# joelle-o-world/dusp

Measured on AMD Instinct MI355X. Metric: rendered Msamples/sec (whole node) + HBM GB/s fraction, 1024-voice 48kHz, higher is better.
Workload: dtype f64; 1 GPU; configs[2] per-voice: 1024 voices/GPU x Multiply(Osc(10k), Ramp(T,1,0) triggered), 60s @48000 Hz, every voice's PCM written; voices_per_gpu=1024, voices_total=1024, n_samples=2880000, engine=fused, parallelism=voices sharded over 1 GPU(s), no collective

## Files before the change

dusp_amd/csrc/abi_internal.hpp:

```cpp
#pragma once
#include <hip/hip_runtime.h>

#include <algorithm>
#include <cstddef>
#include <cstdint>
#include <exception>
#include <map>
#include <mutex>
#include <new>
#include <stdexcept>
#include <string>
#include <utility>
#include <vector>

#include "../../include/dusp_hip.h"
#include "device_types.hpp"
#include "fused_plan.hpp"
#include "jit_codegen.hpp"
#include "program.hpp"
#include "score_plan.hpp"

namespace dusp {
hipError_t launch_chunk_engine(const ChunkArgs &a, hipStream_t stream);
hipError_t launch_state_init(double *state, const double *init, uint32_t n_slots, uint32_t n_pad, hipStream_t stream);
// ... 113 lines not shown
    DevBuf<int64_t> d_jit_regime;

    static constexpr size_t kCount = 28;

    template <class F>
    void for_each_workspace(F &&f) {
        f("chunk buffers", d_scratch);
        f("rings", d_rings);
        f("unit state", d_state);
        f("segment phases", d_seg);
        f("fused end state", d_fused_state);
        f("voice records", d_recs);
        f("sum-chain records", d_sum_voices);
        f("parked chunks", d_saved_bufs);
        f("parked rings", d_rings_wave);
        f("staging PCM", d_host_out);
        f("staging frames", d_host_frames);
        f("staging PCM frames / peaks", d_host_pcm);
        f("staging PCM frames / peaks", d_host_peaks);
        f("mix sums / gains", d_mix);
        f("mix sums / gains", d_mix_gains);
        f("staging parameters", d_host_par);
        f("staging inputs", d_host_in);
        f("hand-off buffers", d_handoff_init);
        f("hand-off buffers", d_handoff_out);
        f("program constants", d_ops);
        f("program constants", d_out_bufs);
        f("program constants", d_init);
        f("compiled kernel's constants", d_jit_fk);
        f("compiled kernel's constants", d_jit_dk);
        f("compiled kernel's constants", d_jit_scan);
        f("warm-up records", d_warm_records);
        f("warm-up start state", d_warm_init);
        f("column verdicts", d_jit_regime);
    }
    const char *first_overwritten() {
        const char *hit = nullptr;
        for_each_workspace([&](const char *name, auto &buf) {
            if (!hit && !buf.intact()) hit = name;
        });
        return hit;
    }
};
static_assert(sizeof(dusp_workspaces) == dusp_workspaces::kCount * sizeof(DevBuf<char>), "dusp_workspaces holds DevBufs only: update kCount and for_each_workspace");

struct dusp_program : dusp_workspaces {
    dusp_ctx *ctx = nullptr;
    dusp::Program P;
    int engine = DUSP_ENGINE_CHUNK;
    dusp::FusedPlan fused;
    dusp::WavePlan wave;
    std::vector<dusp::SumVoice> h_sum_voices;
    std::vector<double> h_sum_end;
    uint32_t last_n_inst = 0, last_n_pad = 0;
    bool rendered = false;
    std::vector<double> h_state;
    bool h_state_valid = false;
    bool mixed = false;
    std::vector<unsigned> mix_range;
    uint32_t mix_n_inst = 0;
    int requested_engine = DUSP_ENGINE_AUTO;
    bool resumable = false;
    bool persistent = false;
    bool keep_memory = false;
    bool delay_changed = false;
    bool migrate_to_chunk = false;
    int64_t next_clock = 0;
    hipEvent_t ev0 = nullptr, ev1 = nullptr;
    hipStream_t last_stream = nullptr;
    bool jit_ok = false;
    std::string jit_why;
    std::map<std::pair<int, int>, dusp::JitSource> jit_src;
    bool jit_consts_uploaded = false;
    int voice_loop = -1;
    uint64_t jit_table_generation = 0;
    int jit_waves = 0, jit_per_wave = 0;
    unsigned jit_segments = 1;
    bool jit_voices = false;
    bool jit_scan = false;
    bool handoff_ok = false;
    std::string handoff_why;
    unsigned warm_redo_from = 0;
    unsigned char *pin[1] = {nullptr};
    size_t pin_bytes = 0;

    dusp_program() = default;
    dusp_program(const dusp_program &) = delete;
    dusp_program &operator=(const dusp_program &) = delete;
    ~dusp_program() {
        if (ctx) (void)hipSetDevice(ctx->device);
        for_each_workspace([](const char *, auto &buf) { buf.release(); });
        if (pin[0]) (void)hipHostFree(pin[0]);
        if (ev0) (void)hipEventDestroy(ev0);
        if (ev1) (void)hipEventDestroy(ev1);
    }
};

#define CTX_FAIL(ctx, code, msg)  \
    do {                          \
        (ctx)->err = (msg);       \
        return (code);            \
    } while (0)

#define HIP_TRY(ctx, expr)                                                                        \
    do {                                                                                          \
        hipError_t e_ = (expr);                                                                   \
        if (e_ != hipSuccess) {                                                                   \
            (ctx)->err = std::string("HIP error: ") + hipGetErrorString(e_) + " in " + #expr;     \
            return DUSP_ERR_HIP;                                                                  \
        }                                                                                         \
    } while (0)

template <class F>
int guarded(std::string &err, const char *who, F &&body) noexcept {
    try {
        return body();
    } catch (const std::bad_alloc &) {
        try { err = std::string(who) + ": out of host memory"; } catch (...) {}
        return DUSP_ERR_NOMEM;
    } catch (const std::length_error &e) {
        try { err = std::string(who) + ": size out of range (" + e.what() + ")"; } catch (...) {}
        return DUSP_ERR_ARG;
    } catch (const std::exception &e) {
        try { err = std::string(who) + ": " + e.what(); } catch (...) {}
        return DUSP_ERR_ARG;
    } catch (...) {
        try { err = std::string(who) + ": unknown internal error"; } catch (...) {}
        return DUSP_ERR_ARG;
    }
}

inline bool instances_in_range(size_t n_instances) { return n_instances >= 1 && n_instances <= (1u << 24); }
inline bool samples_in_range(size_t n_samples) { return n_samples >= 1 && n_samples <= (1ull << 31); }
inline bool batch_in_range(size_t n_instances, size_t n_samples) { return instances_in_range(n_instances) && samples_in_range(n_samples); }
inline bool channels_in_range(size_t n_channels) { return n_channels >= 1 && n_channels <= 64; }

inline int check_batch(dusp_ctx *ctx, const char *who, size_t n_instances, size_t n_samples) {
    if (!batch_in_range(n_instances, n_samples)) CTX_FAIL(ctx, DUSP_ERR_ARG, std::string(who) + ": n_instances must be in [1, 2^24] and n_samples in [1, 2^31]");
    return DUSP_OK;
}
inline int check_channels(dusp_ctx *ctx, const char *who, size_t n_channels) {
    if (!channels_in_range(n_channels)) CTX_FAIL(ctx, DUSP_ERR_UNSUPPORTED, std::string(who) + ": the outlet must have 1..64 channels");
    return DUSP_OK;
}
inline int check_pcm_format(dusp_ctx *ctx, const char *who, int format, bool allow_planar) {
    if ((format != 0 || !allow_planar) && format != DUSP_PCM_S16 && format != DUSP_PCM_S24 && format != DUSP_PCM_F32)
        CTX_FAIL(ctx, DUSP_ERR_ARG, std::string(who) + ": format must be " + (allow_planar ? "0 (planar f32), " : "") + "DUSP_PCM_S16 (1), DUSP_PCM_S24 (2) or DUSP_PCM_F32 (3)");
// ... 26 lines not shown
```

dusp_amd/csrc/abi_program.hip:

```cpp
#include <cmath>
#include <cstdio>
#include <cstdlib>
#include <cstring>
#include <memory>

#include "abi_internal.hpp"
#include "engine_select.hpp"
#include "jit_engine.hpp"

extern "C" {

static int select_engine(dusp_program *prog) {
    dusp_ctx *ctx = prog->ctx;
    dusp::EngineRequest rq;
    rq.requested = prog->requested_engine;
    rq.resumable = prog->resumable;
    rq.rendered = prog->rendered;
    rq.engine_so_far = prog->engine;
    rq.delay_changed = prog->delay_changed;
    rq.wave_jit = ctx->knobs.wave_jit;
    for (int k = 0; k < dusp::kNumTables; k++) rq.table_set[k] = ctx->table_set[k], rq.table_fx32_ok[k] = ctx->table_fx32_ok[k];
    dusp::EngineChoice choice = dusp::engine_select(prog->P, rq, std::move(prog->wave.ramp_checked));
    prog->fused = std::move(choice.fused);
    prog->wave = std::move(choice.wave);
    prog->persistent = choice.persistent;
    if (choice.error) CTX_FAIL(ctx, choice.error, choice.error_text);
    prog->engine = choice.engine;
    prog->jit_src.clear();
    prog->jit_consts_uploaded = false;
    prog->jit_ok = choice.jit_ok;
    prog->jit_why = std::move(choice.jit_why);
    prog->handoff_ok = choice.handoff_ok;
    prog->handoff_why = std::move(choice.handoff_why);
    return DUSP_OK;
}

static int upload_constants(dusp_program *prog) {
    dusp_ctx *ctx = prog->ctx;
    HIP_TRY(ctx, hipSetDevice(ctx->device));
    const dusp::Program &P = prog->P;
    size_t n_all_ops = P.ops.size();
    for (const auto &w : P.warm_ops) n_all_ops += w.size();
    HIP_TRY(ctx, prog->d_ops.ensure(n_all_ops));
    std::vector<int32_t> out_bufs = P.out_bufs;
    if (prog->engine == DUSP_ENGINE_WAVE) {
        std::vector<dusp::DevOp> ops = P.ops;
        const auto &slot = prog->wave.buf_slot;
        for (size_t k = 0; k < ops.size(); k++) {
            if (ops[k].out_buf >= 0) ops[k].out_buf = slot[(size_t)ops[k].out_buf];
            for (auto &in : ops[k].in)
                if (in.kind == dusp::SRC_BUF && in.idx >= 0 && in.idx < P.n_bufs) in.idx = slot[(size_t)in.idx];
            ops[k].lds_slot = prog->wave.op_state[k];
        }
        for (auto &op : ops)
            if (op.op == dusp::OP_RETRIGGER) op.pad = prog->wave.op_state[(size_t)op.pad];
        for (auto &b : out_bufs) b = slot[(size_t)b];
        std::vector<dusp::DevOp> ordered(ops.size());
        for (size_t at = 0; at < ops.size(); at++) ordered[at] = ops[(size_t)prog->wave.order[at]];
        HIP_TRY(ctx, hipMemcpy(prog->d_ops.p, ordered.data(), ordered.size() * sizeof(dusp::DevOp), hipMemcpyHostToDevice));
    } else
    HIP_TRY(ctx, hipMemcpy(prog->d_ops.p, P.ops.data(), P.ops.size() * sizeof(dusp::DevOp), hipMemcpyHostToDevice));
    n_all_ops = P.ops.size();
    for (const auto &w : P.warm_ops) {
        if (!w.empty())
            HIP_TRY(ctx, hipMemcpy(prog->d_ops.p + n_all_ops, w.data(), w.size() * sizeof(dusp::DevOp), hipMemcpyHostToDevice));
        n_all_ops += w.size();
    }
    HIP_TRY(ctx, prog->d_out_bufs.ensure(out_bufs.size()));
    HIP_TRY(ctx, hipMemcpy(prog->d_out_bufs.p, out_bufs.data(), out_bufs.size() * sizeof(int32_t), hipMemcpyHostToDevice));
    if (!P.init_state.empty()) {
        HIP_TRY(ctx, prog->d_init.ensure(P.init_state.size()));
        HIP_TRY(ctx, hipMemcpy(prog->d_init.p, P.init_state.data(), P.init_state.size() * sizeof(double), hipMemcpyHostToDevice));
    }
    return DUSP_OK;
}

// ... 44 lines not shown
    const dusp::Program &P = prog->P;
    bool same = next.g.units.size() == P.g.units.size() && next.ops.size() == P.ops.size() && next.n_bufs == P.n_bufs &&
                next.ring_samples == P.ring_samples && next.out_bufs == P.out_bufs && next.g.n_params == P.g.n_params &&
                next.g.sample_rate == P.g.sample_rate && next.init_state.size() == P.init_state.size() &&
                next.dev_rings.size() == P.dev_rings.size();
    for (size_t k = 0; same && k < P.g.units.size(); k++) same = next.g.units[k].op == P.g.units[k].op && next.g.units[k].n_out == P.g.units[k].n_out;
    for (size_t k = 0; same && k < P.ops.size(); k++) {
        const dusp::DevOp &a = P.ops[k], &b = next.ops[k];
        same = a.op == b.op && a.unit == b.unit && a.out_buf == b.out_buf && a.state_slot == b.state_slot && a.ring_base == b.ring_base &&
               a.ring_len == b.ring_len && a.n_in == b.n_in;
        for (int j = 0; same && j < dusp::kMaxIn; j++)
            same = (a.in[j].kind == dusp::SRC_BUF) == (b.in[j].kind == dusp::SRC_BUF) && (a.in[j].kind != dusp::SRC_BUF || a.in[j].idx == b.in[j].idx);
    }
    if (!same) CTX_FAIL(ctx, DUSP_ERR_ARG, "dusp_program_continue: the descriptor does not describe the circuit this program was built from");
    if (next.g.clock0 != prog->next_clock)
        CTX_FAIL(ctx, DUSP_ERR_STATE, "dusp_program_continue: descriptor clock " + std::to_string(next.g.clock0) + " does not follow the rendered clock " +
                                          std::to_string(prog->next_clock));
    const bool persistent = next.ring_samples != 0 || !next.feed_forward;
    if (persistent && !(prog->resumable && (prog->engine == DUSP_ENGINE_CHUNK || prog->engine == DUSP_ENGINE_WAVE)))
        CTX_FAIL(ctx, DUSP_ERR_STATE, "dusp_program_continue: a circuit with delay lines / feedback has to be built with DUSP_ENGINE_RESUMABLE");
    const int engine_before = prog->engine;
    bool delay_changed = prog->delay_changed;
    for (size_t k = 0; k < P.ops.size(); k++)
        if (P.ops[k].op == dusp::OP_DELAY) {
            const dusp::DevOperand &a = P.ops[k].in[1], &b = next.ops[k].in[1];
            if (a.kind != b.kind || a.idx != b.idx || std::memcmp(&a.cval, &b.cval, sizeof(float)) != 0) delay_changed = true;
        }
    struct Before {
        dusp::Program P; bool delay_changed; int engine;
    } before{std::move(prog->P), prog->delay_changed, prog->engine};
    prog->P = std::move(next);
    prog->delay_changed = delay_changed;
    if (int rc = finish_build(prog)) {
        const std::string why = ctx->err;
        prog->P = std::move(before.P);
        prog->delay_changed = before.delay_changed;
        const int requested = prog->requested_engine;
        prog->requested_engine = before.engine;
        const int back = finish_build(prog);
        prog->requested_engine = requested;
        ctx->err = back == DUSP_OK ? why : why + " (and the previous program could not be restored: " + ctx->err + ")";
        return rc;
    }
    prog->keep_memory = persistent;
    if (persistent && engine_before == DUSP_ENGINE_WAVE && prog->engine == DUSP_ENGINE_CHUNK) prog->migrate_to_chunk = true;
    return DUSP_OK;
    });
}

void dusp_program_destroy(dusp_program *prog) {
    if (!prog) return;
    (void)hipSetDevice(prog->ctx->device);
    if (prog->rendered && prog->ev1) (void)hipEventSynchronize(prog->ev1);
    (void)hipStreamSynchronize(prog->ctx->stream);
    delete prog;
}

int dusp_program_info_get(const dusp_program *prog, dusp_program_info *info) {
    if (!prog || !info) return DUSP_ERR_ARG;
    std::memset(info, 0, sizeof *info);
    const dusp::Graph &g = prog->P.g;
    info->sample_rate = (uint32_t)g.sample_rate;
    info->chunk_size = (uint32_t)g.chunk;
    info->n_units = (uint32_t)g.units.size();
    info->n_out_channels = (uint32_t)prog->P.out_bufs.size();
    info->n_params = (uint32_t)g.n_params;
    info->engine = (uint32_t)prog->engine;
    info->n_device_ops = (uint32_t)prog->P.ops.size();
    info->n_inputs = (uint32_t)g.n_inputs;
    if (prog->engine == DUSP_ENGINE_FUSED) std::snprintf(info->shape, sizeof info->shape, "%s", prog->fused.shape.c_str());
    if (prog->engine == DUSP_ENGINE_WAVE && prog->jit_ok && (prog->jit_waves || !prog->rendered))
    {
        const int at = std::snprintf(info->shape, sizeof info->shape, "%s, compiled kernel: %d units, %dx%d", prog->P.feed_forward ? "feed-forward" : "feedback",
                                     (int)prog->P.ops.size(), prog->jit_waves, prog->jit_per_wave);
        if (at > 0 && (size_t)at < sizeof info->shape && (prog->jit_voices || prog->jit_segments > 1)) {
            if (prog->jit_voices && prog->jit_segments > 1) std::snprintf(info->shape + at, sizeof info->shape - (size_t)at, ", loop, %u seg", prog->jit_segments);
            else if (prog->jit_voices) std::snprintf(info->shape + at, sizeof info->shape - (size_t)at, ", voice loop");
            else if (prog->warm_redo_from) std::snprintf(info->shape + at, sizeof info->shape - (size_t)at, ", %u seg, redo@%u", prog->jit_segments, prog->warm_redo_from);
            else std::snprintf(info->shape + at, sizeof info->shape - (size_t)at, ", %u seg", prog->jit_segments);
        } else if (at > 0 && (size_t)at < sizeof info->shape && prog->jit_scan)
            std::snprintf(info->shape + at, sizeof info->shape - (size_t)at, ", scan");
    }
    else if (prog->engine == DUSP_ENGINE_WAVE && prog->jit_ok)
        std::snprintf(info->shape, sizeof info->shape, "%s, %d chunk buffers in LDS (kernel compiling)", prog->P.feed_forward ? "feed-forward" : "feedback", prog->wave.n_slots);
    else if (prog->engine == DUSP_ENGINE_WAVE)
        std::snprintf(info->shape, sizeof info->shape, "%s, %d chunk buffers in LDS", prog->P.feed_forward ? "feed-forward" : "feedback", prog->wave.n_slots);
    if (prog->engine == DUSP_ENGINE_CHUNK && !prog->P.warm_ops.empty() && !prog->handoff_ok && !prog->handoff_why.empty())
        std::snprintf(info->shape, sizeof info->shape, "warm-up, then not compiled: %.34s", prog->handoff_why.c_str());
    if (prog->engine == DUSP_ENGINE_CHUNK && prog->handoff_ok && prog->jit_waves)
        std::snprintf(info->shape, sizeof info->shape, "%d warm-up chunks here, then compiled kernel: %d units, %dx%d", (int)prog->P.warm_ops.size(), (int)prog->P.ops.size(),
                      prog->jit_waves, prog->jit_per_wave);
    return DUSP_OK;
}

int dusp_state_download(dusp_program *prog, size_t instance, size_t unit, double *out, size_t cap) {
    if (!prog) return DUSP_ERR_ARG;
    dusp_ctx *ctx = prog->ctx;
    return guarded(ctx->err, "dusp_state_download", [&]() -> int {
    if (!prog->rendered) CTX_FAIL(ctx, DUSP_ERR_STATE, "dusp_state_download: nothing has been rendered yet");
    if (prog->mixed) CTX_FAIL(ctx, DUSP_ERR_STATE, "dusp_state_download: the last render was a mix (dusp_render_host_mix, dusp_render_host_score): unit state describes its last tile only");
    const dusp::Graph &g = prog->P.g;
    if (unit >= g.units.size() || instance >= prog->last_n_inst || !out)
        CTX_FAIL(ctx, DUSP_ERR_ARG, "dusp_state_download: unit / instance out of range");
    HIP_TRY(ctx, hipSetDevice(ctx->device));
    HIP_TRY(ctx, hipEventSynchronize(prog->ev1));
    const dusp::UnitDesc &u = g.units[unit];
// ... 117 lines not shown
```

dusp_amd/csrc/abi_render.hip:

```cpp
#include <cstring>

#include "abi_internal.hpp"
#include "jit_plan.hpp"
#include "render_plan.hpp"
#include "ring_windows.hpp"

static int check_tables(dusp_program *prog) {
    dusp_ctx *ctx = prog->ctx;
    for (const auto &u : prog->P.g.units)
        if (u.op == dusp::OP_OSC || u.op == dusp::OP_MULTI_OSC || u.op == dusp::OP_SHAPE) {
            const int w = (int)u.attrs[0];
            if (!ctx->d_tables || !ctx->table_set[w])
                CTX_FAIL(ctx, DUSP_ERR_STATE, "render: wave table " + std::to_string(w) + " has not been uploaded (dusp_table_upload)");
            if (ctx->table_len != (uint32_t)prog->P.g.sample_rate + 1)
                CTX_FAIL(ctx, DUSP_ERR_STATE, "render: wave table length != sample_rate + 1");
        }
    return DUSP_OK;
}


hipError_t zero_rings(dusp_program *prog, uint32_t n_pad, uint32_t n_chunks, bool instance_major, hipStream_t stream) {
    const dusp::Program &P = prog->P;
    float *rings = prog->d_rings.p;
    const size_t total = (size_t)P.ring_samples;
// ... 49 lines not shown
    a.table_stride = prog->ctx->table_stride;
    a.flags = flags;
    a.n_warm = (uint32_t)P.warm_ops.size();
    for (uint32_t k = 0, at = a.n_ops; k < a.n_warm; k++) {
        a.warm_first[k] = at;
        a.warm_n[k] = (uint32_t)P.warm_ops[k].size();
        at += a.warm_n[k];
    }
    return a;
}


int check_guards(dusp_program *prog, hipStream_t stream) {
    dusp_ctx *ctx = prog->ctx;
    if (!g_guard_bytes) return DUSP_OK;
    HIP_TRY(ctx, hipStreamSynchronize(stream));
    const char *hit = prog->first_overwritten();
    if (!hit && ctx->tables_guarded && ctx->d_tables && !guard_intact((const char *)ctx->d_tables + sizeof(float) * dusp::kNumTables * ctx->table_stride)) hit = "lookup tables";
    if (hit) CTX_FAIL(ctx, DUSP_ERR_HIP, std::string("render: a kernel wrote past the end of a device buffer (") + hit + "): guard bytes overwritten");
    return DUSP_OK;
}

struct RenderCall {
    uint32_t n_inst, n_chunks, n_pad;
    size_t n_samples;
    const float *d_params, *d_inputs;
    float *d_out;
    hipStream_t stream;
};

static size_t chunk_workspace_floats(const dusp::Program &P, uint32_t rows) { return (size_t)std::max(1, P.n_bufs) * dusp::kChunk * rows; }
static size_t state_workspace_doubles(const dusp::Program &P, uint32_t n_pad) { return std::max<size_t>(1, P.init_state.size()) * n_pad; }
static size_t ring_workspace_floats(const dusp::Program &P, uint32_t n_pad) { return std::max<size_t>(1, (size_t)P.ring_samples) * n_pad; }

static int clear_chunk_memory(dusp_program *prog, uint32_t n_pad, hipStream_t stream) {
    dusp_ctx *ctx = prog->ctx;
    HIP_TRY(ctx, hipMemsetAsync(prog->d_scratch.p, 0, chunk_workspace_floats(prog->P, n_pad) * sizeof(float), stream));
    if (prog->P.ring_samples) HIP_TRY(ctx, hipMemsetAsync(prog->d_rings.p, 0, (size_t)prog->P.ring_samples * n_pad * sizeof(float), stream));
    return DUSP_OK;
}

static int render_sum_chain(dusp_program *prog, const RenderCall &c, dusp::FusedLaunch &L, const ChainWindow *window) {
    dusp_ctx *ctx = prog->ctx;
    const uint32_t n_inst = c.n_inst;
    hipStream_t stream = c.stream;
    if (!L.table_fx32_ok) CTX_FAIL(ctx, DUSP_ERR_UNSUPPORTED, "render: wave table has entries below 2^-20; build this program with DUSP_ENGINE_CHUNK");
    const int gb = dusp::sumchain_group_blocks(n_inst, c.n_samples, ctx->n_cus);
    if (!gb) CTX_FAIL(ctx, DUSP_ERR_UNSUPPORTED, "render: too many samples for the fused sum chain; use DUSP_ENGINE_CHUNK");
    if (window) {
        L.chain_first = window->first;
        L.chain_init = window->init;
        L.chain_raw = window->raw;
    }
    dusp::build_sum_voices(prog->fused, (uint32_t)prog->P.g.sample_rate, gb, L.chain_first + (uint64_t)c.n_chunks * dusp::kChunk, prog->h_sum_voices, prog->h_sum_end);
    HIP_TRY(ctx, prog->d_sum_voices.ensure(prog->h_sum_voices.size()));
    HIP_TRY(ctx, hipMemcpyAsync(prog->d_sum_voices.p, prog->h_sum_voices.data(), prog->h_sum_voices.size() * sizeof(dusp::SumVoice), hipMemcpyHostToDevice, stream));
    std::vector<double> end((size_t)prog->fused.n_state_words * n_inst);
    for (int w = 0; w < prog->fused.n_state_words; w++)
        for (uint32_t i = 0; i < n_inst; i++) end[(size_t)w * n_inst + i] = prog->h_sum_end[(size_t)w];
    HIP_TRY(ctx, hipMemcpyAsync(prog->d_fused_state.p, end.data(), end.size() * sizeof(double), hipMemcpyHostToDevice, stream));
    HIP_TRY(ctx, hipStreamSynchronize(stream));
    HIP_TRY(ctx, hipEventRecord(prog->ev0, stream));
    HIP_TRY(ctx, dusp::launch_sumchain(prog->fused, L, prog->d_sum_voices.p, gb, stream));
    HIP_TRY(ctx, hipEventRecord(prog->ev1, stream));
    return DUSP_OK;
}

static int render_fused(dusp_program *prog, const RenderCall &c, const ChainWindow *window) {
    dusp_ctx *ctx = prog->ctx;
    dusp::FusedLaunch L{};
    L.params = c.d_params;
    L.tables = ctx->d_tables;
    L.table_stride = ctx->table_stride;
    L.out = c.d_out;
    L.n_inst = c.n_inst;
    L.n_samples = c.n_samples;
    L.n_chunks = c.n_chunks;
    L.sample_rate = (uint32_t)prog->P.g.sample_rate;
    L.n_cus = ctx->n_cus;
    L.table_antisym = ctx->table_antisym[prog->fused.table_id];
    L.table_finite = ctx->table_finite[prog->fused.table_id];
    L.table_fx32_ok = ctx->table_fx32_ok[prog->fused.table_id];
    L.table_delta = ctx->table_delta[prog->fused.table_id];
    L.table_form = ctx->table_form[prog->fused.table_id];
    L.knobs = ctx->knobs;
    HIP_TRY(ctx, prog->d_recs.ensure(c.n_inst));
    L.recs = prog->d_recs.p;
    HIP_TRY(ctx, prog->d_fused_state.ensure((size_t)std::max(1, prog->fused.n_state_words) * c.n_inst));
    L.end_state = prog->d_fused_state.p;
    if (prog->fused.kind == dusp::FUSED_SUMCHAIN) {
        if (int rc = render_sum_chain(prog, c, L, window)) return rc;
    } else {
        HIP_TRY(ctx, hipEventRecord(prog->ev0, c.stream));
        HIP_TRY(ctx, dusp::launch_fused(prog->fused, L, c.stream));
        HIP_TRY(ctx, hipEventRecord(prog->ev1, c.stream));
    }
    finish_render(prog, c.n_inst, c.n_pad, c.n_chunks);
    return DUSP_OK;
}

static int render_wave_interpreter(dusp_program *prog, const RenderCall &c) {
    dusp_ctx *ctx = prog->ctx;
    const dusp::Program &P = prog->P;
    const uint32_t n_inst = c.n_inst, n_pad = c.n_pad, n_chunks = c.n_chunks;
    hipStream_t stream = c.stream;
    HIP_TRY(ctx, prog->d_state.ensure(state_workspace_doubles(P, n_pad)));
    dusp::WaveArgs w{};
    w.ops = prog->d_ops.p;
    w.out_bufs = prog->d_out_bufs.p;
    w.params = c.d_params;
    w.tables = ctx->d_tables;
    w.inputs = c.d_inputs;
    w.out = c.d_out;
    w.state = prog->d_state.p;
    w.init_state = prog->d_init.p;
    w.n_samples = c.n_samples;
    w.n_ops = (uint32_t)P.ops.size();
    w.n_out = (uint32_t)P.out_bufs.size();
    w.n_inst = n_inst;
    w.n_pad = n_pad;
    w.n_bufs = (uint32_t)prog->wave.n_slots;
    w.n_state_ops = (uint32_t)prog->wave.n_state_ops;
    w.n_groups = n_chunks;
    w.sample_rate = (uint32_t)P.g.sample_rate;
    w.table_stride = ctx->table_stride;
    w.vec4_ok = (c.n_samples % 4 == 0) && (((uintptr_t)c.d_out & 15) == 0);
    w.lds_table_id = prog->wave.lds_table_id;
    w.clock0 = (uint64_t)P.g.clock0;
    w.has_filter = prog->wave.has_filter ? 1u : 0u;
    w.scratch_bytes = (uint32_t)prog->wave.scratch_bytes;
    w.ring_events = prog->wave.ring_events ? 1u : 0u;
    w.ext_units = (uint32_t)prog->wave.ext_units;
    w.n_params = (uint32_t)P.g.n_params;
    w.ring_samples = (uint64_t)P.ring_samples;
    const bool resume = prog->keep_memory;
    if (resume && n_inst != prog->last_n_inst) CTX_FAIL(ctx, DUSP_ERR_STATE, "render: the instance count cannot change while a program is being continued");
    if (P.ring_samples && !resume) {
        HIP_TRY(ctx, prog->d_rings.ensure(ring_workspace_floats(P, n_pad)));
        HIP_TRY(ctx, zero_rings(prog, n_pad, n_chunks, true, stream));
    }
    w.rings = prog->d_rings.p;
    w.resume = resume ? 1u : 0u;
    w.save_bufs = (prog->resumable && prog->persistent) ? 1u : 0u;
    if (w.save_bufs) {
        HIP_TRY(ctx, prog->d_saved_bufs.ensure(chunk_workspace_floats(P, n_inst)));
// ... 175 lines not shown
```

dusp_amd/csrc/fused_engine.hip:

```cpp
#include <hip/hip_runtime.h>

#include <type_traits>

#include "device_types.hpp"
#include "fused_device.hpp"
#include "fused_plan.hpp"
#include "repeat_add.hpp"

namespace dusp {

namespace {

template <bool FASTDIV>
__device__ __forceinline__ float ramp_value(const FusedArgs &A, double tn, double dy) {
    const double tt = fmin(tn, A.r_d);
    double q;
    if (FASTDIV) {
        q = tt * A.r_rcp;
        const double rem = fma(-q, A.r_d, tt);
        q = fma(rem, A.r_rcp, q);
    } else
        q = tt / A.r_d;
    return (float)(A.r_y0 + q * dy);
}
// ... 13 lines not shown
    for (int c = 1; c < 4; ++c) P[c] = addmod(P[c - 1], rc.Fm, rc.S);
}

}

__global__ void dusp_fused_prepare(FusedArgs A, OscRec *recs) {
    const uint32_t inst = blockIdx.x * blockDim.x + threadIdx.x;
    if (inst >= A.n_inst) return;
    const uint32_t sr = A.sample_rate;
    const double srd = (double)sr;
    OscRec rc;
    double fd = (double)operand_value(A.f, A.params, A.n_inst, inst);
    rc.bad = !(fabs(fd) <= 3.0e38);
    if (rc.bad) fd = 0.0;
    if (fabs(fd) >= srd) fd = fmod(fd, srd);
    int E = 0;
    if (fd != 0.0) E = min(E, lsb_exponent(fd));
    if (A.phase0 != 0.0) E = min(E, lsb_exponent(A.phase0));
    const int Emin = -(62 - (32 - __builtin_clz(sr)));
    if (E < Emin) E = Emin;
    rc.E = E;
    rc.u = ldexp(1.0, E);
    rc.S = (uint64_t)sr << (-E);
    const long long F = (long long)rint(ldexp(fd, -E));
    rc.Fm = F >= 0 ? (uint64_t)F : rc.S - (uint64_t)(-F);
    if (rc.Fm >= rc.S) rc.Fm -= rc.S;
    rc.P0 = (uint64_t)rint(ldexp(A.phase0, -E));
    if (rc.P0 >= rc.S) rc.P0 %= rc.S;
    rc.step4 = mulmod(rc.Fm, 4, rc.S);
    rc.step256 = mulmod(rc.Fm, kChunk, rc.S);
    rc.segstep = mulmod(rc.Fm, (uint64_t)A.seg_groups * kChunk, rc.S);
    rc.gain = A.gain.kind == SRC_PARAM || A.gain.kind == SRC_CONST ? operand_value(A.gain, A.params, A.n_inst, inst) : 1.f;
    rc.pad = 0;
    recs[inst] = rc;

    const uint64_t T_end = (uint64_t)A.n_chunks * kChunk;
    double phase_end = (double)addmod(rc.P0, mulmod(rc.Fm, T_end, rc.S), rc.S) * rc.u;
    if (rc.bad) phase_end = __builtin_nan("");
    A.end_state[(size_t)A.osc_state_word * A.n_inst + inst] = phase_end;
    if (A.ramp_state_word >= 0) {
        const double t_end = A.r_playing ? fmin(A.r_t0 + (double)T_end, A.r_d) : A.r_t0;
        const bool playing_end = A.r_playing && (A.r_t0 + (double)T_end <= A.r_d);
        A.end_state[(size_t)A.ramp_state_word * A.n_inst + inst] = t_end;
        A.end_state[(size_t)(A.ramp_state_word + 1) * A.n_inst + inst] = playing_end ? 1.0 : 0.0;
    }
    if (A.shape_state_word >= 0) {
        const double t_end = A.s_playing ? repeat_add(A.s_t0, A.s_c, T_end) : A.s_t0;
        A.end_state[(size_t)A.shape_state_word * A.n_inst + inst] = t_end;
        A.end_state[(size_t)(A.shape_state_word + 1) * A.n_inst + inst] = A.s_playing ? 1.0 : 0.0;
        A.end_state[(size_t)(A.shape_state_word + 2) * A.n_inst + inst] = (A.s_finished || (T_end > 0 && t_end > srd)) ? 1.0 : 0.0;
    }
}

template <int KIND, int TBL, int R, bool FASTDIV, bool FINITE, int BLOCK>
__global__ void __launch_bounds__(BLOCK) dusp_fused_kernel(FusedArgs A, const OscRec *__restrict__ recs) {
    extern __shared__ __attribute__((aligned(16))) float lds_table[];
    Table<TBL> table;
    table.g = A.table;
    table.h = lds_table;
    table.N = A.sample_rate + 1;
    table.M = A.sample_rate / 2;
    table.form = make_table_form(A.table_form, A.sample_rate);
    if (TBL == 1) load_half_table<BLOCK>(lds_table, A.table, A.sample_rate);
    const uint32_t lane = threadIdx.x & 63u;
    constexpr uint32_t waves_per_block = BLOCK / 64;
    constexpr int RS = R < 4 ? R : 4;
    const uint32_t n_blk = (A.n_inst + R - 1) / R;
    const uint64_t n_items = (uint64_t)n_blk * A.n_seg;
    const uint64_t total_waves = (uint64_t)gridDim.x * waves_per_block;
    const double srd = (double)A.sample_rate;
    const uint32_t sr = A.sample_rate;
    const double dy = A.r_y1 - A.r_y0;
    const uint32_t n_full = A.vec4_ok ? (uint32_t)(A.n_samples / kChunk) : 0u;

    for (uint64_t item = (uint64_t)blockIdx.x * waves_per_block + (threadIdx.x >> 6); item < n_items; item += total_waves) {
        const uint32_t blk = A.seg_major ? (uint32_t)(item / A.n_seg) : (uint32_t)(item % n_blk);
        const uint32_t seg = A.seg_major ? (uint32_t)(item % A.n_seg) : (uint32_t)(item / n_blk);
        const uint32_t g0 = seg * A.seg_groups;
        const uint32_t g1 = min(g0 + A.seg_groups, A.n_groups);
        const uint32_t gm = max(g0, min(g1, n_full));
        const uint64_t t_start = (uint64_t)g0 * kChunk;

        uint32_t inst[R];
        int e_min = 0;
        bool any_bad = false;
#pragma unroll
        for (int r = 0; r < R; ++r) {
            inst[r] = min(blk * R + r, A.n_inst - 1);
            e_min = min(e_min, recs[inst[r]].E);
            any_bad = any_bad || recs[inst[r]].bad;
        }
        float *const row0 = A.out + t_start + lane * 4;
        const double tn0 = A.r_t0 + (A.r_playing ? (double)(t_start + lane * 4 + 1) : 0.0);
        const double tn_step = A.r_playing ? (double)kChunk : 0.0;
        const double tn_c = A.r_playing ? 1.0 : 0.0;
        double tn;
        const double st0 = (KIND == FUSED_OSC_SHAPE && A.s_playing) ? repeat_add(A.s_t0, A.s_c, t_start) : A.s_t0;
        double st;
        auto ramp4 = [&](float (&rv)[4]) {
            if (KIND == FUSED_OSC_SHAPE) {
                if (!A.s_playing) {
#pragma unroll
                    for (int c = 0; c < 4; ++c) rv[c] = shape_value(A, st, srd);
                } else {
                    long long T, ce;
                    int K;
                    if (linear_run(st, A.s_c, kChunk, T, ce, K)) {
                        T += (long long)(lane * 4) * ce;
#pragma unroll
                        for (int c = 0; c < 4; ++c) {
                            T += ce;
                            rv[c] = shape_value(A, ldexp((double)T, K - 52), srd);
                        }
                        st = ldexp((double)(T + (long long)(kChunk - 4 - lane * 4) * ce), K - 52);
                    } else {
                        double t = repeat_add(st, A.s_c, (uint64_t)lane * 4);
#pragma unroll
                        for (int c = 0; c < 4; ++c) rv[c] = shape_value(A, t = t + A.s_c, srd);
                        st = __shfl(t, 63, 64);
                    }
                }
            }
            if (KIND == FUSED_OSC_RAMP) {
                rv[0] = ramp_value<FASTDIV>(A, tn, dy);
#pragma unroll
                for (int c = 1; c < 4; ++c) rv[c] = ramp_value<FASTDIV>(A, tn + tn_c * c, dy);
                tn += tn_step;
            }
// ... 185 lines not shown
                run(gm, g1, std::false_type{});
            }
        } else {
            for (int sub = 0; sub < R; sub += RS) {
                double ph[RS][4], D[RS];
                size_t roff[RS];
                float gain[RS];
                bool bad[RS];
#pragma unroll
                for (int r = 0; r < RS; ++r) {
                    const OscRec rc = recs[inst[sub + r]];
                    uint64_t P[4];
                    start_phase(rc, seg, lane, P);
                    for (int c = 0; c < 4; ++c) ph[r][c] = (double)P[c] * rc.u;
                    D[r] = (double)rc.step256 * rc.u;
                    roff[r] = (size_t)inst[sub + r] * A.n_samples;
                    gain[r] = rc.gain;
                    bad[r] = rc.bad;
                }
                tn = tn0;
            st = st0;
                float *row = row0;
                auto run = [&](uint32_t ga, uint32_t gb, auto vec) {
                    for (uint32_t g = ga; g < gb; ++g) {
                        float rv[4] = {1.f, 1.f, 1.f, 1.f};
                        ramp4(rv);
#pragma unroll
                        for (int r = 0; r < RS; ++r) {
                            float v[4];
#pragma unroll
                            for (int c = 0; c < 4; ++c) {
                                const uint32_t idx = (uint32_t)(int)ph[r][c];
                                const double fraction = ph[r][c] - (double)(int)idx;
                                float ta, tb;
                                table.pair(idx, ta, tb);
                                float x = (float)((double)ta * (1.0 - fraction) + (double)tb * fraction);
                                if (bad[r]) x = 0.f;
                                v[c] = finish(x, rv[c], gain[r]);
                                ph[r][c] += D[r];
                                if (ph[r][c] >= srd) ph[r][c] -= srd;
                            }
                            store4<decltype(vec)::value>(row + roff[r], v, (uint64_t)g * kChunk + lane * 4, A.n_samples);
                        }
                        row += kChunk;
                    }
                };
                run(g0, gm, std::true_type{});
                run(gm, g1, std::false_type{});
            }
        }
    }
}

template <int KIND, int TBL, int R, bool FASTDIV, bool FINITE, int BLOCK>
static hipError_t launch_one(const FusedArgs &A, const OscRec *recs, int grid, size_t lds_bytes, hipStream_t stream) {
    auto kernel = dusp_fused_kernel<KIND, TBL, R, FASTDIV, FINITE, BLOCK>;
    if (lds_bytes > 65536) {
        hipError_t e = hipFuncSetAttribute((const void *)kernel, hipFuncAttributeMaxDynamicSharedMemorySize, (int)lds_bytes);
        if (e != hipSuccess) return e;
    }
    hipLaunchKernelGGL(kernel, dim3((unsigned)grid), dim3(BLOCK), lds_bytes, stream, A, recs);
    return hipGetLastError();
}

hipError_t launch_fused(const FusedPlan &plan, const FusedLaunch &L, hipStream_t stream) {
    FusedArgs A{};
    A.params = L.params;
    A.table = L.tables + (size_t)plan.table_id * L.table_stride;
    A.out = L.out;
    A.end_state = L.end_state;
    A.n_samples = L.n_samples;
    A.n_inst = L.n_inst;
    A.n_groups = (uint32_t)((L.n_samples + kChunk - 1) / kChunk);
    A.sample_rate = L.sample_rate;
    A.n_chunks = L.n_chunks;
    A.f = plan.f;
    A.gain = plan.gain;
    if (plan.kind != FUSED_OSC_GAIN) A.gain.kind = -1;
    A.phase0 = plan.phase0;
    A.r_d = plan.r_d; A.r_y0 = plan.r_y0; A.r_y1 = plan.r_y1; A.r_t0 = plan.r_t0; A.r_rcp = plan.r_rcp;
    A.r_playing = plan.r_playing;
    A.r_fastdiv = plan.r_fastdiv;
    A.vec4_ok = (L.n_samples % 4 == 0) && (((uintptr_t)L.out & 15) == 0);
    A.osc_state_word = 0;
    A.ramp_state_word = plan.kind == FUSED_OSC_RAMP ? 1 : -1;
    A.shape_state_word = plan.kind == FUSED_OSC_SHAPE ? 1 : -1;
    if (plan.kind == FUSED_OSC_SHAPE) {
        A.s_table = L.tables + (size_t)plan.s_table_id * L.table_stride;
        A.s_t0 = plan.s_t0; A.s_c = plan.s_c; A.s_min = plan.s_min; A.s_max = plan.s_max;
        A.s_left = plan.s_left; A.s_right = plan.s_right;
        A.s_left_is_shape = plan.s_left_is_shape; A.s_right_is_shape = plan.s_right_is_shape;
        A.s_playing = plan.s_playing; A.s_finished = plan.s_finished;
    }
    auto ordinary = [](double y) { return y == 0.0 || (std::fabs(y) >= 9.3e-10 && std::fabs(y) <= 1.1e18); };
    A.r_scale_ok = plan.kind == FUSED_OSC_RAMP && ordinary(plan.r_y0) && ordinary(plan.r_y1) && plan.r_d <= 1.1e12 && (plan.r_t0 == 0.0 || plan.r_t0 >= 1.0) &&
                           L.knobs.fused_fx32 != 2
                       ? 1 : 0;
    A.fx32_ok = L.table_fx32_ok && L.knobs.fused_fx32 ? 1 : 0;
    A.table_delta = L.knobs.fused_fx32 == 1 ? L.table_delta : 0;
    A.seg_major = L.knobs.fused_segmajor;

    int tbl = (L.table_antisym && L.sample_rate % 2 == 0) ? 1 : 0;
    if (L.table_form >= TABLE_FORM_SAW && L.table_form <= TABLE_FORM_TRIANGLE) tbl = 2;
    A.table_form = L.table_form;
    if (L.knobs.fused_table_global) tbl = 0;
    const size_t lds_bytes = tbl == 1 ? half_table_lds_bytes(L.sample_rate) : 0;
    if (lds_bytes > 160 * 1024) tbl = 0;

    int R = L.knobs.fused_R;
    if (R != 1 && R != 4 && R != 8) R = 4;
    const int block = tbl == 1 ? 1024 : 256;
    const int grid = tbl == 1 ? L.n_cus : L.n_cus * 8;
    const uint64_t total_waves = (uint64_t)grid * (block / 64);
    const uint64_t n_blk = (A.n_inst + R - 1) / R;
    auto cut = [&](uint64_t per_wave, uint64_t &n_seg) {
// ... 40 lines not shown
```

dusp_amd/csrc/fused_plan.hpp:

```cpp
#pragma once
#include <cmath>
#include <string>
#include <vector>

#include "device_types.hpp"
#include "program.hpp"

namespace dusp {

enum : int { FUSED_OSC = 0, FUSED_OSC_RAMP = 1, FUSED_OSC_GAIN = 2, FUSED_SUMCHAIN = 3, FUSED_OSC_SHAPE = 4 };

struct FusedPlan {
    std::string shape, why;
    int kind = FUSED_OSC;
    int table_id = 0;
    DevOperand f{}, gain{};
    double phase0 = 0;
    double r_d = 1, r_y0 = 0, r_y1 = 0, r_t0 = 0, r_rcp = 1;
    int r_playing = 0, r_fastdiv = 0;
    int s_table_id = 0, s_playing = 0, s_finished = 0, s_left_is_shape = 0, s_right_is_shape = 0;
    double s_t0 = 0, s_c = 0, s_left = 0, s_right = 0;
    float s_min = 0, s_max = 1;
    std::vector<double> sum_f, sum_phase0;
    std::vector<int> sum_units;
    bool sum_all_int = false;
    int sum_env = 0;
    std::vector<float> sum_gain;
    std::vector<int> sum_ramp_units;
    int n_state_words = 0;
    std::vector<int> unit_state_first, unit_state_count;
};

struct OscRec {
    uint64_t S, Fm, P0;
    uint64_t step4, step256, segstep;
    double u;
    int32_t E, bad;
    float gain, pad;
};

struct SumVoice {
    uint64_t B0, bs, step4, step256, Fm;
    float gain;
    uint32_t pad;
};

struct SumArgs {
    const SumVoice *voices;
    const float *table;
    float *out;
    uint64_t n_samples, S;
    double inv_S, inv_sr;
    uint32_t n_voices, n_inst, n_groups, n_blocks, sample_rate, vec4_ok;
    double r_d, r_y0, r_y1, r_t0;
    int32_t r_playing, r_fastdiv;
    const float *init;
    uint32_t first_block, raw;
};

struct WaveArgs {
    const DevOp *ops;
    const int32_t *out_bufs;
    const float *params;
    const float *tables;
    float *out;
    double *state;
    const double *init_state;
    uint64_t n_samples;
    uint32_t n_ops, n_out, n_inst, n_pad, n_bufs, n_groups, sample_rate, table_stride, vec4_ok;
    int32_t lds_table_id;
    uint32_t table_bytes, wave_bytes;
    float *rings;
    uint64_t ring_samples, clock0;
    uint32_t has_filter, scratch_bytes;
    const float *inputs;
    uint32_t n_state_ops;
    uint32_t ring_events;
    uint32_t ext_units;
    uint32_t n_seg, seg_groups;
    uint32_t pass_mode;
    uint32_t pass_level;
    unsigned long long *seg_sum, *seg_start;
    int32_t max_osc_level, pad4;
    float *saved_bufs;
    uint32_t save_bufs, resume;
    uint32_t n_params, param_bytes;
};

inline size_t wave_param_bytes(size_t n_params) { return n_params && n_params <= 2048 ? (n_params * 4 + 15) & ~(size_t)15 : 0; }
inline size_t wave_lds_bytes(size_t n_bufs, size_t n_state_ops, size_t scratch_bytes) {
    return (n_bufs * 1024 + n_state_ops * 96 + (scratch_bytes ? scratch_bytes + 16 : 0) + 15) & ~(size_t)15;
}

struct WavePlan {
    bool ok = false, has_filter = false;
    int scratch_bytes = 0;
    std::vector<int> order;
    std::vector<int> buf_slot;
    std::vector<int> op_state;
    int n_slots = 0, n_state_ops = 0;
    int ext_units = 0;
    bool ring_events = false;
    bool splittable = false;
    bool splittable_but_for_filters = false;
    int max_osc_level = 0;
    std::vector<int> osc_level;
    std::vector<int> ramp_fastdiv;
    struct RampChecked { double d, t0; bool ok; };
    std::vector<RampChecked> ramp_checked;
    int lds_table_id = -1;
    std::string why;
// ... 561 lines not shown
```

dusp_amd/csrc/sumchain_engine.hip:

```cpp
#include <hip/hip_runtime.h>

#include "device_types.hpp"
#include "fused_device.hpp"
#include "fused_plan.hpp"

namespace dusp {

template <int TBL, bool INT, int GB, bool FINITE, int BLOCK, int ENV>
__global__ void __launch_bounds__(BLOCK) dusp_sumchain_kernel(SumArgs A) {
    extern __shared__ __attribute__((aligned(16))) float lds_table[];
    Table<TBL> table;
    table.g = A.table;
    table.h = lds_table;
    table.N = A.sample_rate + 1;
    table.M = A.sample_rate / 2;
    if (TBL == 1) load_half_table<BLOCK>(lds_table, A.table, A.sample_rate);

    const uint32_t lane = threadIdx.x & 63u;
    constexpr uint32_t waves_per_block = BLOCK / 64;
    const uint64_t n_items = (uint64_t)A.n_inst * A.n_blocks;
    const uint64_t total_waves = (uint64_t)gridDim.x * waves_per_block;
    const uint32_t sr = A.sample_rate;
    const uint32_t n_full = A.first_block * GB + (A.vec4_ok ? (uint32_t)(A.n_samples / kChunk) : 0u);

    for (uint64_t item = (uint64_t)blockIdx.x * waves_per_block + (threadIdx.x >> 6); item < n_items; item += total_waves) {
        const uint32_t blk = (uint32_t)(item % A.n_blocks) + A.first_block;
        const uint32_t inst = (uint32_t)(item / A.n_blocks);
        const uint32_t g0 = blk * GB;
        const size_t row_at = (size_t)inst * A.n_samples + (size_t)(g0 - A.first_block * GB) * kChunk + lane * 4;
        float acc[GB][4];
#pragma unroll
        for (int g = 0; g < GB; ++g)
            for (int c = 0; c < 4; ++c) acc[g][c] = 0.f;
        if (A.init) {
#pragma unroll
            for (int g = 0; g < GB; ++g)
                if (g0 + g < n_full) {
                    const f32x4 v = *(const f32x4 *)(A.init + row_at + (size_t)g * kChunk);
                    acc[g][0] = v[0]; acc[g][1] = v[1]; acc[g][2] = v[2]; acc[g][3] = v[3];
                } else if (g0 + g < A.n_groups) {
                    const uint64_t t = (uint64_t)(g0 + g - A.first_block * GB) * kChunk + lane * 4;
                    for (int c = 0; c < 4; ++c)
                        if (t + c < A.n_samples) acc[g][c] = A.init[row_at + (size_t)g * kChunk + c];
                }
        }
        float env[ENV == 2 ? GB : 1][4];
        if (ENV == 2) {
            const double dy = A.r_y1 - A.r_y0, rcp = 1.0 / A.r_d;
#pragma unroll
            for (int g = 0; g < (ENV == 2 ? GB : 1); ++g)
#pragma unroll
                for (int c = 0; c < 4; ++c) {
                    const uint64_t n = (uint64_t)(g0 + g) * kChunk + lane * 4 + c;
                    const double tt = A.r_playing ? fmin(A.r_t0 + (double)(n + 1), A.r_d) : A.r_t0;
                    double q;
                    if (A.r_fastdiv) {
                        q = tt * rcp;
                        q = fma(fma(-q, A.r_d, tt), rcp, q);
                    } else
                        q = tt / A.r_d;
                    env[g][c] = (float)(A.r_y0 + q * dy);
                }
        }

        for (uint32_t j = 0; j < A.n_voices; ++j) {
            const SumVoice rc = A.voices[j];
            if (INT) {
                const uint32_t f = (uint32_t)(rc.Fm >> 32), s4 = (uint32_t)(rc.step4 >> 32), s256 = (uint32_t)(rc.step256 >> 32);
                const uint32_t base = mod_u32((uint32_t)(rc.B0 >> 32) + blk * (uint32_t)(rc.bs >> 32), sr, A.inv_sr);
                uint32_t idx[4];
                idx[0] = mod_u32(base + lane * s4, sr, A.inv_sr);
#pragma unroll
                for (int c = 1; c < 4; ++c) {
                    idx[c] = idx[c - 1] + f;
                    idx[c] = min(idx[c], idx[c] - sr);
                }
#pragma unroll
                for (int g = 0; g < GB; ++g)
#pragma unroll
                    for (int c = 0; c < 4; ++c) {
                        float v = table.at(idx[c]);
                        if (ENV == 1) v = v * rc.gain;
                        if (ENV == 2) v = v * env[g][c];
                        acc[g][c] = acc[g][c] + v;
                        idx[c] += s256;
                        idx[c] = min(idx[c], idx[c] - sr);
                    }
            } else {
                const uint64_t base = mod_u64(rc.B0 + (uint64_t)blk * rc.bs, A.S, A.inv_S);
                uint64_t P = mod_u64(base + (uint64_t)lane * rc.step4, A.S, A.inv_S);
                uint32_t I[4], F[4];
#pragma unroll
                for (int c = 0; c < 4; ++c) {
                    I[c] = (uint32_t)(P >> 32);
                    F[c] = (uint32_t)P;
                    P += rc.Fm;
                    if (P >= A.S) P -= A.S;
                }
                const uint32_t dI = (uint32_t)(rc.step256 >> 32), dF = (uint32_t)rc.step256;
#pragma unroll
                for (int g = 0; g < GB; ++g)
#pragma unroll
                    for (int c = 0; c < 4; ++c) {
                        float ta, tb;
                        table.pair(I[c], ta, tb);
                        const double wb = (double)F[c];
                        const double wa = 4294967296.0 - wb;
                        const float x = (float)((double)ta * wa + (double)tb * wb);
                        float v = ldexpf(x, -32);
                        if (ENV == 1) v = v * rc.gain;
                        if (ENV == 2) v = v * env[g][c];
                        acc[g][c] = acc[g][c] + v;
                        const uint32_t f2 = F[c] + dF;
                        uint32_t i2 = I[c] + dI + (f2 < F[c] ? 1u : 0u);
                        i2 = min(i2, i2 - sr);
                        F[c] = f2;
                        I[c] = i2;
                    }
            }
        }
        float *row = A.out + row_at;
#pragma unroll
        for (int g = 0; g < GB; ++g) {
            const uint32_t gg = g0 + g;
            if (gg >= A.n_groups) break;
            float v[4];
            for (int c = 0; c < 4; ++c) v[c] = A.raw ? acc[g][c] : fix_out<FINITE>(acc[g][c]);
            if (gg < n_full)
                store4<true>(row, v, 0, A.n_samples);
            else
                store4<false>(row, v, (uint64_t)(gg - A.first_block * GB) * kChunk + lane * 4, A.n_samples);
            row += kChunk;
        }
    }
}

template <int TBL, bool INT, int GB, bool FINITE, int BLOCK, int ENV>
static hipError_t launch_sum(const SumArgs &A, int grid, size_t lds_bytes, hipStream_t stream) {
    auto kernel = dusp_sumchain_kernel<TBL, INT, GB, FINITE, BLOCK, ENV>;
    if (lds_bytes > 65536) {
        hipError_t e = hipFuncSetAttribute((const void *)kernel, hipFuncAttributeMaxDynamicSharedMemorySize, (int)lds_bytes);
        if (e != hipSuccess) return e;
    }
    hipLaunchKernelGGL(kernel, dim3((unsigned)grid), dim3(BLOCK), lds_bytes, stream, A);
    return hipGetLastError();
}

hipError_t launch_sumchain(const FusedPlan &plan, const FusedLaunch &L, const SumVoice *d_voices, int gb, hipStream_t stream) {
    SumArgs A{};
    A.voices = d_voices;
    A.table = L.tables + (size_t)plan.table_id * L.table_stride;
    A.out = L.out;
    A.n_samples = L.n_samples;
    A.S = (uint64_t)L.sample_rate << 32;
    A.inv_S = 1.0 / (double)A.S;
    A.inv_sr = 1.0 / (double)L.sample_rate;
    A.n_voices = (uint32_t)plan.sum_f.size();
    A.n_inst = L.n_inst;
    A.first_block = (uint32_t)(L.chain_first / ((uint64_t)gb * kChunk));
    A.init = L.chain_init;
    A.raw = L.chain_raw ? 1u : 0u;
    const uint32_t window_groups = (uint32_t)((L.n_samples + kChunk - 1) / kChunk);
    A.n_groups = A.first_block * (uint32_t)gb + window_groups;
    A.n_blocks = (window_groups + gb - 1) / gb;
    A.sample_rate = L.sample_rate;
    A.vec4_ok = (L.n_samples % 4 == 0) && (((uintptr_t)L.out & 15) == 0);
    A.r_d = plan.r_d;
    A.r_y0 = plan.r_y0;
    A.r_y1 = plan.r_y1;
    A.r_t0 = plan.r_t0;
    A.r_playing = plan.r_playing;
    A.r_fastdiv = plan.r_fastdiv;

    const bool tbl = L.table_antisym && L.sample_rate % 2 == 0 && half_table_lds_bytes(L.sample_rate) <= 160 * 1024;
    const size_t lds_bytes = tbl ? half_table_lds_bytes(L.sample_rate) : 0;
    const int grid = tbl ? L.n_cus : L.n_cus * 8;
    const bool finite = L.table_finite && plan.sum_env == 0;
    const bool use_int = plan.sum_all_int && ((uint64_t)A.first_block + A.n_blocks) * L.sample_rate < (1ull << 32);

#define DUSP_S5(TB, IN, G, FIN, EN) \
    return TB ? launch_sum<1, IN, G, FIN, 1024, EN>(A, grid, lds_bytes, stream) : launch_sum<0, IN, G, FIN, 256, EN>(A, grid, 0, stream)
#define DUSP_S4(TB, IN, G, FIN) \
    do { if (plan.sum_env == 2) { DUSP_S5(TB, IN, G, FIN, 2); } if (plan.sum_env == 1) { DUSP_S5(TB, IN, G, FIN, 1); } DUSP_S5(TB, IN, G, FIN, 0); } while (0)
#define DUSP_S3(IN, G) \
    do { if (finite) { DUSP_S4(tbl, IN, G, true); } DUSP_S4(tbl, IN, G, false); } while (0)
    if (gb == 8) {
        if (use_int) DUSP_S3(true, 8);
        DUSP_S3(false, 8);
    }
    if (use_int) DUSP_S3(true, 4);
    DUSP_S3(false, 4);
#undef DUSP_S3
#undef DUSP_S4
#undef DUSP_S5
}

}
```

Baseline: 1.529 million Msamples/s.

## Cache sumchain voice uploads, deal work items across blocks, use magic-number modulo

Sumchain voice records and end-state rows are now uploaded only when the gb, instance count, end sample or buffers change, and the per-render host stream synchronize is replaced by an event. The fused and sumchain kernels deal work items across blocks wave-major when there are fewer items than wave slots, and sumchain blocks with no work exit before loading the LDS table. The sumchain integer modulo by sample rate now uses a multiply-high magic number instead of a double reciprocal. Together these aim to cut host overhead on repeated renders and spread a small item count over more CUs, at the cost of cache-invalidation complexity.

After: 1.385 million Msamples/s. -9.4%, worse.

```diff
diff --git a/dusp_amd/csrc/abi_internal.hpp b/dusp_amd/csrc/abi_internal.hpp
--- a/dusp_amd/csrc/abi_internal.hpp
+++ b/dusp_amd/csrc/abi_internal.hpp
@@ -189,6 +189,16 @@
     dusp::WavePlan wave;
     std::vector<dusp::SumVoice> h_sum_voices;
     std::vector<double> h_sum_end;
+    struct SumCache {
+        bool records = false, end = false;
+        int gb = 0;
+        uint32_t n_inst = 0;
+        uint64_t end_sample = 0;
+        const void *d_voices = nullptr, *d_state = nullptr;
+    } sum_cache;
+    std::vector<double> h_sum_rows;
+    hipEvent_t sum_uploaded = nullptr;
+    bool sum_upload_pending = false;
     uint32_t last_n_inst = 0, last_n_pad = 0;
     bool rendered = false;
     std::vector<double> h_state;
@@ -230,6 +240,7 @@
         if (pin[0]) (void)hipHostFree(pin[0]);
         if (ev0) (void)hipEventDestroy(ev0);
         if (ev1) (void)hipEventDestroy(ev1);
+        if (sum_uploaded) (void)hipEventDestroy(sum_uploaded);
     }
 };
 
diff --git a/dusp_amd/csrc/abi_program.hip b/dusp_amd/csrc/abi_program.hip
--- a/dusp_amd/csrc/abi_program.hip
+++ b/dusp_amd/csrc/abi_program.hip
@@ -22,6 +22,7 @@
     for (int k = 0; k < dusp::kNumTables; k++) rq.table_set[k] = ctx->table_set[k], rq.table_fx32_ok[k] = ctx->table_fx32_ok[k];
     dusp::EngineChoice choice = dusp::engine_select(prog->P, rq, std::move(prog->wave.ramp_checked));
     prog->fused = std::move(choice.fused);
+    prog->sum_cache = {};
     prog->wave = std::move(choice.wave);
     prog->persistent = choice.persistent;
     if (choice.error) CTX_FAIL(ctx, choice.error, choice.error_text);
@@ -172,6 +173,7 @@
     if (!prog) return;
     (void)hipSetDevice(prog->ctx->device);
     if (prog->rendered && prog->ev1) (void)hipEventSynchronize(prog->ev1);
+    if (prog->sum_upload_pending) (void)hipEventSynchronize(prog->sum_uploaded);
     (void)hipStreamSynchronize(prog->ctx->stream);
     delete prog;
 }
diff --git a/dusp_amd/csrc/abi_render.hip b/dusp_amd/csrc/abi_render.hip
--- a/dusp_amd/csrc/abi_render.hip
+++ b/dusp_amd/csrc/abi_render.hip
@@ -125,17 +125,39 @@
         L.chain_init = window->init;
         L.chain_raw = window->raw;
     }
-    dusp::build_sum_voices(prog->fused, (uint32_t)prog->P.g.sample_rate, gb, L.chain_first + (uint64_t)c.n_chunks * dusp::kChunk, prog->h_sum_voices, prog->h_sum_end);
-    HIP_TRY(ctx, prog->d_sum_voices.ensure(prog->h_sum_voices.size()));
-    HIP_TRY(ctx, hipMemcpyAsync(prog->d_sum_voices.p, prog->h_sum_voices.data(), prog->h_sum_voices.size() * sizeof(dusp::SumVoice), hipMemcpyHostToDevice, stream));
-    std::vector<double> end((size_t)prog->fused.n_state_words * n_inst);
-    for (int w = 0; w < prog->fused.n_state_words; w++)
-        for (uint32_t i = 0; i < n_inst; i++) end[(size_t)w * n_inst + i] = prog->h_sum_end[(size_t)w];
-    HIP_TRY(ctx, hipMemcpyAsync(prog->d_fused_state.p, end.data(), end.size() * sizeof(double), hipMemcpyHostToDevice, stream));
-    HIP_TRY(ctx, hipStreamSynchronize(stream));
+    const uint64_t end_sample = L.chain_first + (uint64_t)c.n_chunks * dusp::kChunk;
+    HIP_TRY(ctx, prog->d_sum_voices.ensure(prog->fused.sum_f.size()));
+    dusp_program::SumCache &cache = prog->sum_cache;
+    const bool have_records = cache.records && cache.gb == gb && cache.d_voices == prog->d_sum_voices.p;
+    const bool have_end = have_records && cache.end && cache.end_sample == end_sample && cache.n_inst == n_inst && cache.d_state == prog->d_fused_state.p;
+    if (!have_end) {
+        if (prog->sum_upload_pending) {
+            HIP_TRY(ctx, hipEventSynchronize(prog->sum_uploaded));
+            prog->sum_upload_pending = false;
+        }
+        if (!prog->sum_uploaded) HIP_TRY(ctx, hipEventCreateWithFlags(&prog->sum_uploaded, hipEventDisableTiming));
+        cache.records = have_records;
+        cache.end = false;
+        dusp::build_sum_voices(prog->fused, (uint32_t)prog->P.g.sample_rate, gb, end_sample, prog->h_sum_voices, prog->h_sum_end);
+        if (!have_records)
+            HIP_TRY(ctx, hipMemcpyAsync(prog->d_sum_voices.p, prog->h_sum_voices.data(), prog->h_sum_voices.size() * sizeof(dusp::SumVoice), hipMemcpyHostToDevice, stream));
+        std::vector<double> &rows = prog->h_sum_rows;
+        rows.resize((size_t)prog->fused.n_state_words * n_inst);
+        for (int w = 0; w < prog->fused.n_state_words; w++)
+            for (uint32_t i = 0; i < n_inst; i++) rows[(size_t)w * n_inst + i] = prog->h_sum_end[(size_t)w];
+        HIP_TRY(ctx, hipMemcpyAsync(prog->d_fused_state.p, rows.data(), rows.size() * sizeof(double), hipMemcpyHostToDevice, stream));
+        HIP_TRY(ctx, hipEventRecord(prog->sum_uploaded, stream));
+        prog->sum_upload_pending = true;
+    }
     HIP_TRY(ctx, hipEventRecord(prog->ev0, stream));
     HIP_TRY(ctx, dusp::launch_sumchain(prog->fused, L, prog->d_sum_voices.p, gb, stream));
     HIP_TRY(ctx, hipEventRecord(prog->ev1, stream));
+    cache.records = cache.end = true;
+    cache.gb = gb;
+    cache.n_inst = n_inst;
+    cache.end_sample = end_sample;
+    cache.d_voices = prog->d_sum_voices.p;
+    cache.d_state = prog->d_fused_state.p;
     return DUSP_OK;
 }
 
@@ -164,6 +186,7 @@
     if (prog->fused.kind == dusp::FUSED_SUMCHAIN) {
         if (int rc = render_sum_chain(prog, c, L, window)) return rc;
     } else {
+        prog->sum_cache = {};
         HIP_TRY(ctx, hipEventRecord(prog->ev0, c.stream));
         HIP_TRY(ctx, dusp::launch_fused(prog->fused, L, c.stream));
         HIP_TRY(ctx, hipEventRecord(prog->ev1, c.stream));
diff --git a/dusp_amd/csrc/fused_engine.hip b/dusp_amd/csrc/fused_engine.hip
--- a/dusp_amd/csrc/fused_engine.hip
+++ b/dusp_amd/csrc/fused_engine.hip
@@ -89,7 +89,7 @@
     }
 }
 
-template <int KIND, int TBL, int R, bool FASTDIV, bool FINITE, int BLOCK>
+template <int KIND, int TBL, int R, bool FASTDIV, bool FINITE, int BLOCK, bool DEAL>
 __global__ void __launch_bounds__(BLOCK) dusp_fused_kernel(FusedArgs A, const OscRec *__restrict__ recs) {
     extern __shared__ __attribute__((aligned(16))) float lds_table[];
     Table<TBL> table;
@@ -110,7 +110,8 @@
     const double dy = A.r_y1 - A.r_y0;
     const uint32_t n_full = A.vec4_ok ? (uint32_t)(A.n_samples / kChunk) : 0u;
 
-    for (uint64_t item = (uint64_t)blockIdx.x * waves_per_block + (threadIdx.x >> 6); item < n_items; item += total_waves) {
+    for (uint64_t item = DEAL ? (uint64_t)(threadIdx.x >> 6) * gridDim.x + blockIdx.x : (uint64_t)blockIdx.x * waves_per_block + (threadIdx.x >> 6); item < n_items;
+         item += total_waves) {
         const uint32_t blk = A.seg_major ? (uint32_t)(item / A.n_seg) : (uint32_t)(item % n_blk);
         const uint32_t seg = A.seg_major ? (uint32_t)(item % A.n_seg) : (uint32_t)(item / n_blk);
         const uint32_t g0 = seg * A.seg_groups;
@@ -402,15 +403,22 @@
     }
 }
 
-template <int KIND, int TBL, int R, bool FASTDIV, bool FINITE, int BLOCK>
-static hipError_t launch_one(const FusedArgs &A, const OscRec *recs, int grid, size_t lds_bytes, hipStream_t stream) {
-    auto kernel = dusp_fused_kernel<KIND, TBL, R, FASTDIV, FINITE, BLOCK>;
+template <int KIND, int TBL, int R, bool FASTDIV, bool FINITE, int BLOCK, bool DEAL>
+static hipError_t launch_numbered(const FusedArgs &A, const OscRec *recs, int grid, size_t lds_bytes, hipStream_t stream) {
+    auto kernel = dusp_fused_kernel<KIND, TBL, R, FASTDIV, FINITE, BLOCK, DEAL>;
     if (lds_bytes > 65536) {
         hipError_t e = hipFuncSetAttribute((const void *)kernel, hipFuncAttributeMaxDynamicSharedMemorySize, (int)lds_bytes);
         if (e != hipSuccess) return e;
     }
     hipLaunchKernelGGL(kernel, dim3((unsigned)grid), dim3(BLOCK), lds_bytes, stream, A, recs);
     return hipGetLastError();
+}
+
+template <int KIND, int TBL, int R, bool FASTDIV, bool FINITE, int BLOCK>
+static hipError_t launch_one(const FusedArgs &A, const OscRec *recs, int grid, size_t lds_bytes, hipStream_t stream) {
+    const uint64_t n_items = (uint64_t)((A.n_inst + R - 1) / R) * A.n_seg, slots = (uint64_t)grid * (BLOCK / 64);
+    return n_items < slots ? launch_numbered<KIND, TBL, R, FASTDIV, FINITE, BLOCK, true>(A, recs, grid, lds_bytes, stream)
+                           : launch_numbered<KIND, TBL, R, FASTDIV, FINITE, BLOCK, false>(A, recs, grid, lds_bytes, stream);
 }
 
 hipError_t launch_fused(const FusedPlan &plan, const FusedLaunch &L, hipStream_t stream) {
diff --git a/dusp_amd/csrc/fused_plan.hpp b/dusp_amd/csrc/fused_plan.hpp
--- a/dusp_amd/csrc/fused_plan.hpp
+++ b/dusp_amd/csrc/fused_plan.hpp
@@ -50,13 +50,27 @@
     const float *table;
     float *out;
     uint64_t n_samples, S;
-    double inv_S, inv_sr;
+    double inv_S;
     uint32_t n_voices, n_inst, n_groups, n_blocks, sample_rate, vec4_ok;
     double r_d, r_y0, r_y1, r_t0;
     int32_t r_playing, r_fastdiv;
     const float *init;
     uint32_t first_block, raw;
-};
+    uint32_t sr_magic, pad;
+};
+
+#if defined(__HIPCC__)
+__host__ __device__
+#endif
+inline uint32_t mod_magic(uint32_t m) { return (uint32_t)((1ull << 32) / m); }
+#if defined(__HIPCC__)
+__host__ __device__
+#endif
+inline uint32_t mod_mulhi(uint32_t x, uint32_t m, uint32_t magic) {
+    const uint32_t q = (uint32_t)(((uint64_t)x * magic) >> 32);
+    const uint32_t r = x - q * m;
+    return r >= m ? r - m : r;
+}
 
 struct WaveArgs {
     const DevOp *ops;
diff --git a/dusp_amd/csrc/sumchain_engine.hip b/dusp_amd/csrc/sumchain_engine.hip
--- a/dusp_amd/csrc/sumchain_engine.hip
+++ b/dusp_amd/csrc/sumchain_engine.hip
@@ -14,16 +14,18 @@
     table.h = lds_table;
     table.N = A.sample_rate + 1;
     table.M = A.sample_rate / 2;
-    if (TBL == 1) load_half_table<BLOCK>(lds_table, A.table, A.sample_rate);
 
     const uint32_t lane = threadIdx.x & 63u;
     constexpr uint32_t waves_per_block = BLOCK / 64;
     const uint64_t n_items = (uint64_t)A.n_inst * A.n_blocks;
     const uint64_t total_waves = (uint64_t)gridDim.x * waves_per_block;
+    if ((uint64_t)blockIdx.x >= n_items) return;
+    if (TBL == 1) load_half_table<BLOCK>(lds_table, A.table, A.sample_rate);
+    const uint32_t wave = (uint32_t)__builtin_amdgcn_readfirstlane((int)(threadIdx.x >> 6));
     const uint32_t sr = A.sample_rate;
     const uint32_t n_full = A.first_block * GB + (A.vec4_ok ? (uint32_t)(A.n_samples / kChunk) : 0u);
 
-    for (uint64_t item = (uint64_t)blockIdx.x * waves_per_block + (threadIdx.x >> 6); item < n_items; item += total_waves) {
+    for (uint64_t item = (uint64_t)wave * gridDim.x + blockIdx.x; item < n_items; item += total_waves) {
         const uint32_t blk = (uint32_t)(item % A.n_blocks) + A.first_block;
         const uint32_t inst = (uint32_t)(item / A.n_blocks);
         const uint32_t g0 = blk * GB;
@@ -67,9 +69,9 @@
             const SumVoice rc = A.voices[j];
             if (INT) {
                 const uint32_t f = (uint32_t)(rc.Fm >> 32), s4 = (uint32_t)(rc.step4 >> 32), s256 = (uint32_t)(rc.step256 >> 32);
-                const uint32_t base = mod_u32((uint32_t)(rc.B0 >> 32) + blk * (uint32_t)(rc.bs >> 32), sr, A.inv_sr);
+                const uint32_t base = mod_mulhi((uint32_t)(rc.B0 >> 32) + blk * (uint32_t)(rc.bs >> 32), sr, A.sr_magic);
                 uint32_t idx[4];
-                idx[0] = mod_u32(base + lane * s4, sr, A.inv_sr);
+                idx[0] = mod_mulhi(base + lane * s4, sr, A.sr_magic);
 #pragma unroll
                 for (int c = 1; c < 4; ++c) {
                     idx[c] = idx[c - 1] + f;
@@ -154,7 +156,6 @@
     A.n_samples = L.n_samples;
     A.S = (uint64_t)L.sample_rate << 32;
     A.inv_S = 1.0 / (double)A.S;
-    A.inv_sr = 1.0 / (double)L.sample_rate;
     A.n_voices = (uint32_t)plan.sum_f.size();
     A.n_inst = L.n_inst;
     A.first_block = (uint32_t)(L.chain_first / ((uint64_t)gb * kChunk));
@@ -164,6 +165,7 @@
     A.n_groups = A.first_block * (uint32_t)gb + window_groups;
     A.n_blocks = (window_groups + gb - 1) / gb;
     A.sample_rate = L.sample_rate;
+    A.sr_magic = L.sample_rate >= 2 ? mod_magic(L.sample_rate) : 0;
     A.vec4_ok = (L.n_samples % 4 == 0) && (((uintptr_t)L.out & 15) == 0);
     A.r_d = plan.r_d;
     A.r_y0 = plan.r_y0;
@@ -176,7 +178,8 @@
     const size_t lds_bytes = tbl ? half_table_lds_bytes(L.sample_rate) : 0;
     const int grid = tbl ? L.n_cus : L.n_cus * 8;
     const bool finite = L.table_finite && plan.sum_env == 0;
-    const bool use_int = plan.sum_all_int && ((uint64_t)A.first_block + A.n_blocks) * L.sample_rate < (1ull << 32);
+    const bool use_int = plan.sum_all_int && ((uint64_t)A.first_block + A.n_blocks) * L.sample_rate < (1ull << 32) && L.sample_rate >= 2 &&
+                         L.sample_rate <= (1u << 26);
 
 #define DUSP_S5(TB, IN, G, FIN, EN) \
     return TB ? launch_sum<1, IN, G, FIN, 1024, EN>(A, grid, lds_bytes, stream) : launch_sum<0, IN, G, FIN, 256, EN>(A, grid, 0, stream)
```
